# bassamlab/SigmaRL

Measured on AMD Instinct MI355X. Metric: env-steps/sec (agents x envs x steps), CPM scenario, 16 agents (open loop, 32 steps per launch), higher is better.
Workload: dtype f32

## Files before the change

### include/sigmaenv.h

```cpp
#ifndef SIGMAENV_H
#define SIGMAENV_H

#include <stddef.h>
#include <stdint.h>

#ifdef __cplusplus
extern "C" {
#endif

#define SIGMAENV_ABI_VERSION 5

#define SIGMAENV_OK 0
#define SIGMAENV_EINVAL (-22)
#define SIGMAENV_ENOMEM (-12)
#define SIGMAENV_EHIP (-5)
#define SIGMAENV_ENODEV (-19)

#define SIGMAENV_DIST_C2C 0
#define SIGMAENV_DIST_MTV 1

#define SIGMAENV_REW_DISTANCE 1
#define SIGMAENV_REW_TTC 2
#define SIGMAENV_REW_EXACT_SPARSE 4
#define SIGMAENV_REW_HAS_SPARSE 8
// ... 126 lines not shown
                              uint64_t seed, uint64_t counter0, int32_t path_first, int32_t path_count);

int sigmaenv_get(sigmaenv_t* h, sigmaenv_buf_t which, void** dev_ptr, size_t* bytes);

int sigmaenv_set_lanelets(sigmaenv_t* h, int32_t n_lanelets, int32_t max_points, const float* centers, const uint64_t* neighbors);

int sigmaenv_opponent_fill(sigmaenv_t* h, const float* actions);

int sigmaenv_set_slab(sigmaenv_t* h, void* dev_ptr);
int sigmaenv_set_rollout_slab_stride(sigmaenv_t* h, int64_t stride_floats);

int sigmaenv_set_rollout_obs_record(sigmaenv_t* h, float* base, int64_t stride_floats);

int sigmaenv_sync(sigmaenv_t* h);

int sigmaenv_step_time_ms(sigmaenv_t* h, double* avg_ms, int32_t* n_launches);
#define SIGMAENV_KERNEL_STEP 0
#define SIGMAENV_KERNEL_CBF_QP 1
#define SIGMAENV_KERNEL_CBF_MARGIN 2
#define SIGMAENV_KERNEL_MLP32 3
#define SIGMAENV_KERNEL_ACTOR_BF16 4
#define SIGMAENV_KERNEL_COUNT 5
int sigmaenv_kernel_time_ms(sigmaenv_t* h, int32_t kernel_id, double* avg_ms, int32_t* n_launches);

typedef struct sigmaenv_launch_shape {
  int32_t wave_G, wave_wpb, wave_grid, wave_spec, wave_lds_bytes;
  int32_t kern_fastdiv, kern_par, kern_sn, kern_sg, kern_var, kern_mtvs;
  int32_t map_fast_div, pruned_scan;
  int32_t G, block, grid, reset_block, smem_bytes;
  int32_t reserved[2];
} sigmaenv_launch_shape_t;
int sigmaenv_launch_shape(const sigmaenv_t* h, sigmaenv_launch_shape_t* out);

int sigmaenv_trig_selftest(sigmaenv_t* h, int32_t kind, int32_t n, const float* in, float* out);

typedef struct sigmaenv_actor sigmaenv_actor_t;

int sigmaenv_actor_create(int32_t obs_dim, const float* w1, const float* b1, const float* w2, const float* b2, const float* w3, const float* b3,
                          const float* w4, const float* b4, const float* low, const float* high, sigmaenv_actor_t** out);
void sigmaenv_actor_destroy(sigmaenv_actor_t* a);

int sigmaenv_actor_forward(sigmaenv_t* h, sigmaenv_actor_t* a, const float* obs, float* actions, float* log_prob, float* loc_scale, uint64_t seed,
                           uint64_t counter, int32_t deterministic);

typedef struct sigmaenv_mlp32 sigmaenv_mlp32_t;
#define SIGMAENV_MLP32_EXACT 0
#define SIGMAENV_MLP32_SPLIT 1
int sigmaenv_mlp32_set_mode(sigmaenv_mlp32_t* m, int32_t mode);
int sigmaenv_mlp32_get_mode(const sigmaenv_mlp32_t* m);
int sigmaenv_mlp32_create(int32_t n_layers, const int32_t* dims, const float* const* weights, const float* const* biases, sigmaenv_mlp32_t** out);
void sigmaenv_mlp32_destroy(sigmaenv_mlp32_t* m);
int sigmaenv_mlp32_forward(sigmaenv_t* h, sigmaenv_mlp32_t* m, const float* in, int32_t rows, float* out);
int sigmaenv_actor_forward_f32(sigmaenv_t* h, sigmaenv_mlp32_t* m, const float* obs, float* scratch, const float* low, const float* high, float* actions,
                               float* log_prob, float* loc_scale, uint64_t seed, uint64_t counter, int32_t deterministic);

int sigmaenv_mlp32_forward_rows(sigmaenv_t* h, sigmaenv_mlp32_t* m, const float* in, int32_t rows_per_block, int64_t row_stride, int32_t n_blocks, int64_t block_stride,
                                float* out);

int sigmaenv_mlp32_load_device(sigmaenv_t* h, sigmaenv_mlp32_t* m, const float* const* weights_dev, const float* const* biases_dev);
int sigmaenv_actor_load_device(sigmaenv_t* h, sigmaenv_actor_t* a, const float* const* weights_dev, const float* const* biases_dev);

int sigmaenv_mlp32_forward_save(sigmaenv_t* h, sigmaenv_mlp32_t* m, const float* in, int32_t rows_per_block, int64_t row_stride, int32_t n_blocks, int64_t block_stride,
                                float* out, float* acts);
int sigmaenv_mlp32_backward_workspace(const sigmaenv_mlp32_t* m, int64_t rows, uint64_t* n_floats);
int sigmaenv_mlp32_backward(sigmaenv_t* h, sigmaenv_mlp32_t* m, const float* in, int32_t rows_per_block, int64_t row_stride, int32_t n_blocks, int64_t block_stride,
                            const float* acts, const float* dout, float* workspace, float* const* grad_w, float* const* grad_b);
// ... 285 lines not shown
```

### sigmarl_amd/capi.py

```python
from __future__ import annotations

import ctypes as C
import math
import os

ABI_VERSION = 5
DIST_C2C, DIST_MTV = 0, 1
REW_DISTANCE, REW_TTC, REW_EXACT_SPARSE, REW_HAS_SPARSE, REW_CBF, REW_CBF_QP = 1, 2, 4, 8, 16, 32
CBF_MAX_CIRCLES = 4
N_SHORT_TERM = 3
MAX_SHORT_TERM = 8
MAX_NEARING = 4
N_REWARD_INFO = 12

(BUF_STATE, BUF_PREV_POS, BUF_VERTICES, BUF_PATH, BUF_SHORT_TERM, BUF_DIST_REF, BUF_DIST_LEFT, BUF_DIST_RIGHT,
 BUF_DIST_BOUND, BUF_CLOSEST, BUF_DIST_AGENTS, BUF_COL_AGENTS, BUF_COL_FLAGS, BUF_REWARD, BUF_REWARD_INFO, BUF_OBS,
 BUF_NEARING, BUF_DONE, BUF_TIMER, BUF_ACTION, BUF_CBF_NOMINAL) = range(21)

REWARD_INFO_FIELDS = (
    "rew_progress", "rew_reach_goal", "rew_speed", "rew_centerline", "rew_near_other_agents", "rew_near_left_lane",
    "rew_near_right_lane", "rew_collide_other_agents", "rew_collide_lane", "rew_energy_acceleration",
    "rew_energy_steering", "rew_total",
)

# ... 236 lines not shown

_SIGS = {
    "obs_dim": (C.c_int, [C.c_int32]),
    "obs_dim_ex": (C.c_int, [C.c_int32, C.c_int32]),
    "obs_dim_full": (C.c_int, [C.c_int32, C.c_int32, C.c_int32]),
    "n_short_term": (C.c_int, []),
    "create": (C.c_int, [C.POINTER(Config), C.POINTER(Map), C.c_int, C.c_void_p, C.POINTER(C.c_void_p)]),
    "destroy": (None, [C.c_void_p]),
    "last_error": (C.c_char_p, [C.c_void_p]),
    "reset": (C.c_int, [C.c_void_p, C.c_int32, C.c_void_p, C.c_void_p, C.c_void_p, C.c_void_p, C.c_int32]),
    "step": (C.c_int, [C.c_void_p, C.c_void_p]),
    "observe": (C.c_int, [C.c_void_p]),
    "auto_reset": (C.c_int, [C.c_void_p, C.c_uint64, C.c_uint64, C.c_int32, C.c_int32]),
    "get": (C.c_int, [C.c_void_p, C.c_int, C.POINTER(C.c_void_p), C.POINTER(C.c_size_t)]),
    "sync": (C.c_int, [C.c_void_p]),
    "set_lanelets": (C.c_int, [C.c_void_p, C.c_int32, C.c_int32, C.c_void_p, C.c_void_p]),
    "opponent_fill": (C.c_int, [C.c_void_p, C.c_void_p]),
    "set_scenario_lists": (C.c_int, [C.c_void_p, C.c_int32, C.c_void_p, C.c_void_p, C.c_void_p]),
    "cbf_attach": (C.c_int, [C.c_void_p, C.POINTER(CbfConfig), C.c_void_p, C.c_void_p, C.c_int32]),
    "cbf_rewards": (C.c_int, [C.c_void_p, C.c_void_p, C.c_void_p]),
    "cbf_inject_centers": (C.c_int, [C.c_void_p, C.c_void_p]),
    "cbf_qp": (C.c_int, [C.c_void_p, C.c_void_p, C.c_void_p, C.c_void_p, C.c_void_p]),
    "cbf_regroup": (C.c_int, [C.c_void_p]),
    "cbf_get_groups": (C.c_int, [C.c_void_p, C.c_void_p]),
}
_PRODUCT_ONLY = {
    "build_id": (C.c_char_p, []),
    "step_time_ms": (C.c_int, [C.c_void_p, C.POINTER(C.c_double), C.POINTER(C.c_int32)]),
    "kernel_time_ms": (C.c_int, [C.c_void_p, C.c_int32, C.POINTER(C.c_double), C.POINTER(C.c_int32)]),
    "set_slab": (C.c_int, [C.c_void_p, C.c_void_p]),
    "set_rollout_slab_stride": (C.c_int, [C.c_void_p, C.c_int64]),
    "set_rollout_obs_record": (C.c_int, [C.c_void_p, C.c_void_p, C.c_int64]),
    "trig_selftest": (C.c_int, [C.c_void_p, C.c_int32, C.c_int32, C.c_void_p, C.c_void_p]),
    "step_autoreset": (C.c_int, [C.c_void_p, C.c_void_p, C.c_uint64, C.c_uint64, C.c_int32, C.c_int32]),
    "step_autoreset_n": (C.c_int, [C.c_void_p, C.c_void_p, C.c_int32, C.c_int64, C.c_void_p, C.c_int64, C.c_uint64, C.c_uint64, C.c_int32, C.c_int32]),
    "step_autoreset_many": (C.c_int, [C.c_void_p, C.c_int32, C.c_void_p, C.c_void_p, C.c_void_p, C.c_uint64, C.c_int32, C.c_int32]),
    "actor_create": (C.c_int, [C.c_int32] + [C.c_void_p] * 10 + [C.POINTER(C.c_void_p)]),
    "actor_destroy": (None, [C.c_void_p]),
    "actor_forward": (C.c_int, [C.c_void_p, C.c_void_p, C.c_void_p, C.c_void_p, C.c_void_p, C.c_void_p, C.c_uint64, C.c_uint64, C.c_int32]),
    "mlp32_create": (C.c_int, [C.c_int32, C.c_void_p, C.c_void_p, C.c_void_p, C.POINTER(C.c_void_p)]),
    "mlp32_destroy": (None, [C.c_void_p]),
    "mlp32_forward": (C.c_int, [C.c_void_p, C.c_void_p, C.c_void_p, C.c_int32, C.c_void_p]),
    "mlp32_forward_rows": (C.c_int, [C.c_void_p, C.c_void_p, C.c_void_p, C.c_int32, C.c_int64, C.c_int32, C.c_int64, C.c_void_p]),
    "mlp32_set_mode": (C.c_int, [C.c_void_p, C.c_int32]),
    "mlp32_get_mode": (C.c_int, [C.c_void_p]),
    "mlp32_load_device": (C.c_int, [C.c_void_p, C.c_void_p, C.c_void_p, C.c_void_p]),
    "actor_load_device": (C.c_int, [C.c_void_p, C.c_void_p, C.c_void_p, C.c_void_p]),
    "mlp32_forward_save": (C.c_int, [C.c_void_p, C.c_void_p, C.c_void_p, C.c_int32, C.c_int64, C.c_int32, C.c_int64, C.c_void_p, C.c_void_p]),
    "mlp32_backward_workspace": (C.c_int, [C.c_void_p, C.c_int64, C.POINTER(C.c_uint64)]),
    "mlp32_backward": (C.c_int, [C.c_void_p, C.c_void_p, C.c_void_p, C.c_int32, C.c_int64, C.c_int32, C.c_int64, C.c_void_p, C.c_void_p, C.c_void_p, C.c_void_p, C.c_void_p]),
    "mlp32_forward_save_indexed": (C.c_int, [C.c_void_p, C.c_void_p, C.c_void_p, C.c_int32, C.c_int64, C.c_int32, C.c_int64, C.c_void_p, C.c_int32, C.c_void_p, C.c_void_p]),
    "mlp32_backward_indexed": (C.c_int, [C.c_void_p, C.c_void_p, C.c_void_p, C.c_int32, C.c_int64, C.c_int32, C.c_int64, C.c_void_p, C.c_int32, C.c_void_p, C.c_void_p, C.c_void_p,
                                         C.c_void_p, C.c_void_p]),
    "mlp32_forward_rows_pad": (C.c_int, [C.c_void_p, C.c_void_p, C.c_void_p, C.c_int32, C.c_int64, C.c_int32, C.c_int64, C.c_int32, C.c_int32, C.c_void_p]),
    "mlp32_forward_save_indexed_pad": (C.c_int, [C.c_void_p, C.c_void_p, C.c_void_p, C.c_int32, C.c_int64, C.c_int32, C.c_int64, C.c_void_p, C.c_int32, C.c_int32, C.c_int32,
                                                 C.c_void_p, C.c_void_p]),
    "mlp32_backward_indexed_pad": (C.c_int, [C.c_void_p, C.c_void_p, C.c_void_p, C.c_int32, C.c_int64, C.c_int32, C.c_int64, C.c_void_p, C.c_int32, C.c_int32, C.c_int32, C.c_void_p,
                                             C.c_void_p, C.c_void_p, C.c_void_p, C.c_void_p]),
    "ppo_head": (C.c_int, [C.c_void_p, C.POINTER(PpoHeadArgs)]),
    "ppo_head_1d": (C.c_int, [C.c_void_p, C.POINTER(PpoHead1dArgs)]),
    "optim_workspace": (C.c_int, [C.c_void_p, C.POINTER(OptimArgs), C.POINTER(C.c_uint64)]),
    "optim_step": (C.c_int, [C.c_void_p, C.POINTER(OptimArgs)]),
    "mlp32_resolve_mode": (C.c_int, [C.c_void_p, C.c_void_p]),
    "prb_create": (C.c_int, [C.c_void_p, C.c_int64, C.c_double, C.c_double, C.c_double, C.POINTER(C.c_void_p)]),
    "prb_destroy": (None, [C.c_void_p]),
    "prb_extend": (C.c_int, [C.c_void_p, C.c_void_p, C.c_void_p, C.c_int64]),
# ... 119 lines not shown
```

### sigmarl_amd/csrc/sigmaenv.hip

```cpp
#include <hip/hip_runtime.h>

#include <algorithm>
#include <atomic>
#include <cmath>
#include <cstdio>
#include <cstdlib>
#include <cstring>
#include <string>
#include <type_traits>
#include <vector>

#include "sigmaenv_device.h"

using namespace sigmadev;

#ifdef SIGMAENV_PROFILE
#define PROF_TS2(g, tid, k) do { if ((g).dbg_ts2 && (tid) == 0) (g).dbg_ts2[(size_t)blockIdx.x * 16 + (k)] = __builtin_readcyclecounter(); } while (0)
#else
#define PROF_TS2(g, tid, k) do { } while (0)
#endif

#include "../../include/sigmaenv_ref_weights.h"
static_assert(NS >= 1 && NS <= SIGMAENV_MAX_SHORT_TERM, "SIGMAENV_N_SHORT_TERM out of range");
__device__ __constant__ uint32_t W_REF_BITS[NS] = SIGMAENV_W_REF_BITS;
// ... 237 lines not shown
#pragma unroll
    for (int i = 0; i < 4; ++i) e[i] = make_edge(ev[2 * i], ev[2 * i + 1], ev[2 * i + 2], ev[2 * i + 3]);
  }
  r.hit = false;
  boundary_scan<COLLIDE>(lb, nl, lane, cgx, cgy, qv, e, r.dl, r.cp_l, r.hit);
  boundary_scan<COLLIDE>(rb, nr, lane, cgx, cgy, qv, e, r.dr, r.cp_r, r.hit);
  float wh = (float)((double)c.width / 2.0);
  r.dl[0] = r.dl[0] - wh;
  r.dr[0] = r.dr[0] - wh;
}

__device__ __forceinline__ float query_radius(const float* qv, float cgx, float cgy) {
  float R = 0.0f;
#pragma unroll
  for (int q = 0; q < 4; ++q) {
    float ax = qv[2 * q] - cgx, ay = qv[2 * q + 1] - cgy;
    R = fmaxf(R, sqrtf(ax * ax + ay * ay));
  }
  return R * 1.000001f + 1e-6f;
}

__device__ __forceinline__ int nth_set_bit64(unsigned long long m, int c) {
  for (int t = 0; t < c; ++t) m &= (m - 1ull);
  return m ? (__ffsll((long long)m) - 1) : -1;
}
__device__ __forceinline__ bool box_within(const float4 b, float px, float py, float T2) {
  float dx = fmaxf(fmaxf(b.x - px, px - b.z), 0.0f);
  float dy = fmaxf(fmaxf(b.y - py, py - b.w), 0.0f);
  return !((dx * dx + dy * dy) > T2);
}
struct MaskTask {
  int sl, pl, path, k, npt, nch;
  float ax, ay, bx, by;
  unsigned long long nm_tight, nm_near, nm_far;
  int lvl;
  int own;
  const float4* box;
  float px, py, T2;
  unsigned long long rest;
  bool fast;
};
__device__ __forceinline__ void mask_stage1(const DevMap& m, MaskTask& mt, int task, int path, int cp) {
  mt.sl = task / 3; mt.pl = task - mt.sl * 3; mt.path = path;
  const int pl = mt.pl;
  const float* poly = m.center + (size_t)pl * m.poly_stride + (size_t)path * m.P * 2;
  mt.box = m.chunk_box + ((size_t)path * 3 + pl) * m.nch;
  const ulonglong4* neigh = m.chunk_neigh + ((size_t)path * 3 + pl) * m.nch;
  int k = cp - 1;
  k = k < 0 ? 0 : (k > m.P - 2 ? m.P - 2 : k);
  mt.k = k;
  mt.npt = m.n_center[pl * m.n_paths + path];
  const Seg4 sg = load_segment(reinterpret_cast<const float2*>(poly), k);
  mt.ax = sg.ax; mt.ay = sg.ay; mt.bx = sg.bx; mt.by = sg.by;
  const ulonglong4 nm = neigh[k / SIGMAENV_CHUNK];
  mt.nm_tight = nm.x; mt.nm_near = nm.y; mt.nm_far = nm.z;
  mt.own = k / SIGMAENV_CHUNK;
}
template <bool COLLIDE>
__device__ __forceinline__ void mask_stage2(const DevMap& m, const Smem& s, MaskTask& mt, bool stale_first, int N) {
  const int sl = mt.sl, pl = mt.pl, npt = mt.npt;
  if (mt.k > npt - 2) {
    const float* poly = m.center + (size_t)pl * m.poly_stride + (size_t)mt.path * m.P * 2;
    const int k = npt - 2 < 0 ? 0 : npt - 2;
    const Seg4 sg = load_segment(reinterpret_cast<const float2*>(poly), k);
    mt.ax = sg.ax; mt.ay = sg.ay; mt.bx = sg.bx; mt.by = sg.by;
    const ulonglong4 nm = (m.chunk_neigh + ((size_t)mt.path * 3 + pl) * m.nch)[k / SIGMAENV_CHUNK];
    mt.nm_tight = nm.x; mt.nm_near = nm.y; mt.nm_far = nm.z;
    mt.own = k / SIGMAENV_CHUNK;
  }
  const float px = s.st[sl * 8], py = s.st[sl * 8 + 1];
  mt.px = px; mt.py = py;
  const float MARGIN = 1e-4f;
  const float glx = mt.bx - mt.ax, gly = mt.by - mt.ay;
  const float rl2 = __builtin_amdgcn_rcpf(glx * glx + gly * gly);
  float dg;
  {
    const float vx = px - mt.ax, vy = py - mt.ay;
    const float tq = clampf((vx * glx + vy * gly) * rl2, 0.0f, 1.0f);
    const float ex = (mt.ax + glx * tq) - px, ey = (mt.ay + gly * tq) - py;
    dg = __builtin_amdgcn_sqrtf(fmaf(ey, ey, ex * ex)) * 1.000001f + 1e-6f;
  }
  float T = dg;
  if (pl != 0) {
    const bool stale = stale_first && (sl % N == 0);
    const float* qv = stale ? (s.vold + sl * 10) : (s.vnew + sl * 10);
    float w = 0.0f;
#pragma unroll
    for (int j = 0; j < 4; ++j) {
      const float qx = qv[2 * j], qy = qv[2 * j + 1];
      const float vx = qx - mt.ax, vy = qy - mt.ay;
      const float tq = clampf((vx * glx + vy * gly) * rl2, 0.0f, 1.0f);
      const float ex = (mt.ax + glx * tq) - qx, ey = (mt.ay + gly * tq) - qy;
      const float rx = qx - px, ry = qy - py;
      w = fmaxf(w, __builtin_amdgcn_sqrtf(fmaf(ey, ey, ex * ex)) + __builtin_amdgcn_sqrtf(fmaf(ry, ry, rx * rx)));
    }
    T = fmaxf(fmaxf(T, w * 1.000001f + 1e-6f), COLLIDE ? m.rect_radius : 0.0f);
  }
  T += MARGIN;
  mt.T2 = T * T;
  mt.nch = (npt - 1 + SIGMAENV_CHUNK - 1) / SIGMAENV_CHUNK;
  mt.fast = T + dg <= m.neigh_radius_far;
  mt.lvl = mt.fast ? ((T + dg <= m.neigh_radius_tight) ? 0 : ((T + dg <= m.neigh_radius) ? 1 : 2)) : 3;
  mt.rest = mt.fast ? (mt.lvl == 0 ? mt.nm_tight : (mt.lvl == 1 ? mt.nm_near : mt.nm_far)) : 0ull;
}
__device__ __forceinline__ void mask_stage3(const DevMap& m, const Smem& s, MaskTask& mt, int task) {
  const float px = mt.px, py = mt.py, T2 = mt.T2;
  const int nch = mt.nch;
  unsigned long long mk = 0ull;
  unsigned long long rest = mt.rest;
  if (mt.fast && mt.own < nch) { mk |= 1ull << mt.own; rest &= ~(1ull << mt.own); }
  while (rest) {
    int idx[8];
#pragma unroll
    for (int q = 0; q < 8; ++q) { idx[q] = rest ? (__ffsll((long long)rest) - 1) : -1; rest &= rest - 1ull; }
    float4 b[8];
#pragma unroll
    for (int q = 0; q < 8; ++q) b[q] = mt.box[idx[q] < 0 ? 0 : idx[q]];
#pragma unroll
    for (int q = 0; q < 8; ++q) {
      if (idx[q] >= 0 && idx[q] < nch && box_within(b[q], px, py, T2)) mk |= 1ull << idx[q];
    }
  }
  if (!mt.fast) {
    const float4* gbox = m.group_box + ((size_t)mt.path * 3 + mt.pl) * 8;
    unsigned gm = 0u;
#pragma unroll
    for (int gidx = 0; gidx < 8; ++gidx) {
      if (gidx * 8 < nch && box_within(gbox[gidx], px, py, T2)) gm |= 1u << gidx;
    }
    while (gm) {
      const int gidx = __ffs((int)gm) - 1;
      gm &= gm - 1u;
#pragma unroll
      for (int q = 0; q < 8; ++q) {
        const int cidx = gidx * 8 + q;
        if (cidx < nch && box_within(mt.box[cidx], px, py, T2)) mk |= 1ull << cidx;
      }
    }
  }
  s.npts[task] = mt.npt;
  s.cmask[task] = mk;
  uint8_t* cl = s.cand + task * CAND_LIST;
  for (int j = 0; mk && j < CAND_LIST; ++j) {
    cl[j] = (uint8_t)(__ffsll((long long)mk) - 1);
    mk &= mk - 1ull;
  }
}
template <bool COLLIDE>
__device__ inline void scan_mask_task(const DevMap& m, const Smem& s, int task, bool stale_first, int N) {
  MaskTask mt;
  mask_stage1(m, mt, task, s.path[task / 3], s.cp[task]);
  mask_stage2<COLLIDE>(m, s, mt, stale_first, N);
  mask_stage3(m, s, mt, task);
}

// ... 1293 lines not shown
  while (G > 1 && (B + G - 1) / G < 4 * n_cu) G >>= 1;
  return G;
}

#ifdef SIGMAENV_POISON
__global__ void sigma_poison_probe_kernel(unsigned* out) {
  extern __shared__ char probe_smem[];
  if (threadIdx.x == 0) { probe_smem[0] = 1; out[0] = sigma_lds_alloc_units() + (probe_smem[0] ? 0u : 1u); }
}
static int poison_probe(hipStream_t stream) {
  static bool done = false;
  if (done) return SIGMAENV_OK;
  unsigned* d = nullptr;
  unsigned units[2] = {0u, 0u};
  if (hipMalloc((void**)&d, 8) != hipSuccess) return SIGMAENV_ENOMEM;
  hipLaunchKernelGGL(sigma_poison_probe_kernel, dim3(1), dim3(64), 32768, stream, d);
  hipLaunchKernelGGL(sigma_poison_probe_kernel, dim3(1), dim3(64), 16384, stream, d + 1);
  if (hipMemcpyAsync(units, d, 8, hipMemcpyDeviceToHost, stream) != hipSuccess || hipStreamSynchronize(stream) != hipSuccess) { (void)hipFree(d); return SIGMAENV_EHIP; }
  (void)hipFree(d);
  unsigned granule = 0u;
  for (unsigned g : {64u, 128u, 256u, 512u})
    if (units[0] * g >= 32768u && units[0] * g < 32768u + 2048u && units[1] * g >= 16384u && units[1] * g < 16384u + 2048u) granule = g;
  if (granule == 0u) {
    fprintf(stderr, "sigmaenv (poison build): unexpected LDS_ALLOC.LDS_SIZE readings %u / %u for 32768 / 16384 bytes\n", units[0], units[1]);
    return SIGMAENV_EHIP;
  }
  if (hipMemcpyToSymbol(HIP_SYMBOL(sigmadev::sigma_lds_granule), &granule, sizeof(unsigned)) != hipSuccess) return SIGMAENV_EHIP;
  fprintf(stderr, "sigmaenv (poison build): LDS and scratch buffers are poisoned (LDS_SIZE unit = %u bytes)\n", granule);
  done = true;
  return SIGMAENV_OK;
}
#endif

extern "C" int sigmaenv_create(const sigmaenv_config_t* cfg, const sigmaenv_map_t* map, int device_id, void* hip_stream, sigmaenv_t** out) {
  if (!cfg || !map || !out) return SIGMAENV_EINVAL;
  *out = nullptr;
  if (cfg->abi_version != SIGMAENV_ABI_VERSION) return SIGMAENV_EINVAL;
  for (int k = 0; k < 3; ++k) if (cfg->reserved[k] != 0) return SIGMAENV_EINVAL;
  if (cfg->n_points_short_term != 0 && cfg->n_points_short_term != NS) {
    fprintf(stderr, "sigmaenv_create: n_points_short_term = %d, but this library is built for %d (make -C sigmarl_amd/csrc NS=%d)\n", cfg->n_points_short_term, NS, cfg->n_points_short_term);
    return SIGMAENV_EINVAL;
  }
  if (cfg->env_index_base < 0 || !(cfg->obs_noise_level >= 0.0f)) return SIGMAENV_EINVAL;
  if (cfg->n_envs < 1 || cfg->n_agents < 1 || cfg->n_agents > SIGMAENV_MAX_AGENTS) return SIGMAENV_EINVAL;
  if (cfg->n_nearing < 0 || cfg->n_nearing > SIGMAENV_MAX_NEARING || cfg->n_nearing > cfg->n_agents - 1) return SIGMAENV_EINVAL;
  if (cfg->distance_type != SIGMAENV_DIST_C2C && cfg->distance_type != SIGMAENV_DIST_MTV) return SIGMAENV_EINVAL;
  if (map->n_paths < 1 || map->stride_points < 2) return SIGMAENV_EINVAL;
  int n_dev = 0;
  if (hipGetDeviceCount(&n_dev) != hipSuccess || n_dev < 1 || device_id < 0 || device_id >= n_dev) return SIGMAENV_ENODEV;
  if (hipSetDevice(device_id) != hipSuccess) return SIGMAENV_ENODEV;
#ifdef SIGMAENV_POISON
  { const int rcp = poison_probe(reinterpret_cast<hipStream_t>(hip_stream)); if (rcp != SIGMAENV_OK) return rcp; }
#endif
  sigmaenv* h = new sigmaenv();
  h->cfg = *cfg;
  h->device = device_id;
  h->stream = reinterpret_cast<hipStream_t>(hip_stream);
  const int B = h->B = cfg->n_envs, N = h->N = cfg->n_agents, K = h->K = cfg->n_nearing;
  h->D = sigmaenv_obs_dim_full(N, K, cfg->obs_flags);
  if (h->D < 0) { delete h; return SIGMAENV_EINVAL; }
  h->DL = h->D;
  if (cfg->obs_flags != 0) {
    const ObsLayout L(cfg->obs_flags, N, K);
    if (L.D != h->D) { delete h; return SIGMAENV_EINVAL; }
    h->DL = L.DL;
  }
// ... 39 lines not shown
#define ALLOC(ptr, bytes)                                         \
  if ((rc = dev_alloc(h, (void**)&(ptr), (bytes))) != SIGMAENV_OK) { \
    std::string e = h->err;                                       \
    sigmaenv_destroy(h);                                          \
    fprintf(stderr, "sigmaenv_create: %s\n", e.c_str());        \
    return rc;                                                    \
  }
  float *d_c, *d_l, *d_r, *d_y;
  int32_t *d_nc, *d_nl, *d_nr;
  uint8_t* d_loop;
  ALLOC(d_c, hc.size() * 4 * 3); d_l = d_c + hc.size(); d_r = d_l + hc.size();
  ALLOC(d_y, (size_t)np * S * 4);
  ALLOC(d_nc, (size_t)np * 4 * 3); d_nl = d_nc + np; d_nr = d_nl + np;
  ALLOC(d_loop, (size_t)np);
#define H2D(dst, src, bytes)                                                                     \
  if (hipMemcpyAsync((dst), (src), (bytes), hipMemcpyHostToDevice, h->stream) != hipSuccess) {   \
    sigmaenv_destroy(h);                                                                         \
    return SIGMAENV_EHIP;                                                                        \
  }
  H2D(d_c, hc.data(), hc.size() * 4); H2D(d_l, hl.data(), hl.size() * 4); H2D(d_r, hr.data(), hr.size() * 4);
  H2D(d_y, map->yaw, (size_t)np * S * 4);
  H2D(d_nc, map->n_center, (size_t)np * 4); H2D(d_nl, map->n_left, (size_t)np * 4); H2D(d_nr, map->n_right, (size_t)np * 4);
  H2D(d_loop, map->is_loop, (size_t)np);
  int nch = (P - 1 + SIGMAENV_CHUNK - 1) / SIGMAENV_CHUNK;
  int real_nch = 0;
  for (int p = 0; p < np; ++p) {
    const int longest = std::max(map->n_center[p], std::max(map->n_left[p], map->n_right[p]));
    real_nch = std::max(real_nch, (longest - 1 + SIGMAENV_CHUNK - 1) / SIGMAENV_CHUNK);
  }
  bool prune = real_nch <= 64;
  if (const char* e = getenv("SIGMAENV_PRUNE")) prune = prune && atoi(e) != 0;
  float4 *d_box = nullptr, *d_gbox = nullptr;
  std::vector<float4> hb, hg;
  std::vector<ulonglong4> hn;
  ulonglong4* d_neigh = nullptr;
  const float neigh_radius_far = 9.0f * (sqrtf((float)((double)cfg->length / 2.0) * (float)((double)cfg->length / 2.0) +
                                               (float)((double)cfg->width / 2.0) * (float)((double)cfg->width / 2.0)) * 1.00001f + 1e-5f);
  const float neigh_radius_tight = 3.6f * (sqrtf((float)((double)cfg->length / 2.0) * (float)((double)cfg->length / 2.0) +
                                                 (float)((double)cfg->width / 2.0) * (float)((double)cfg->width / 2.0)) * 1.00001f + 1e-5f);
  const float neigh_radius = 6.0f * (sqrtf((float)((double)cfg->length / 2.0) * (float)((double)cfg->length / 2.0) +
                                           (float)((double)cfg->width / 2.0) * (float)((double)cfg->width / 2.0)) * 1.00001f + 1e-5f);
  if (prune) {
    hb.assign((size_t)np * 3 * nch, make_float4(1e30f, 1e30f, -1e30f, -1e30f));
    for (int p = 0; p < np; ++p) {
      const float* polys[3] = {hc.data() + (size_t)p * P * 2, hl.data() + (size_t)p * P * 2, hr.data() + (size_t)p * P * 2};
      const int cnt[3] = {map->n_center[p], map->n_left[p], map->n_right[p]};
      for (int q = 0; q < 3; ++q) {
        for (int k = 0; k + 1 < cnt[q]; ++k) {
          float4& bx = hb[((size_t)p * 3 + q) * nch + k / SIGMAENV_CHUNK];
          for (int e2 = 0; e2 < 2; ++e2) {
            float x = polys[q][2 * (k + e2)], y = polys[q][2 * (k + e2) + 1];
            bx.x = x < bx.x ? x : bx.x; bx.y = y < bx.y ? y : bx.y; bx.z = x > bx.z ? x : bx.z; bx.w = y > bx.w ? y : bx.w;
          }
        }
      }
    }
    ALLOC(d_box, hb.size() * sizeof(float4));
    H2D(d_box, hb.data(), hb.size() * sizeof(float4));
    hg.assign((size_t)np * 3 * 8, make_float4(1e30f, 1e30f, -1e30f, -1e30f));
    for (size_t pq = 0; pq < (size_t)np * 3; ++pq) {
      for (int cidx = 0; cidx < nch; ++cidx) {
        const float4& bx = hb[pq * nch + cidx];
        if (bx.x > bx.z) continue;
        float4& gx = hg[pq * 8 + cidx / 8];
        gx.x = bx.x < gx.x ? bx.x : gx.x; gx.y = bx.y < gx.y ? bx.y : gx.y; gx.z = bx.z > gx.z ? bx.z : gx.z; gx.w = bx.w > gx.w ? bx.w : gx.w;
      }
    }
    ALLOC(d_gbox, hg.size() * sizeof(float4));
    H2D(d_gbox, hg.data(), hg.size() * sizeof(float4));
    hn.assign((size_t)np * 3 * nch, make_ulonglong4(0ull, 0ull, 0ull, 0ull));
    for (size_t pq = 0; pq < (size_t)np * 3; ++pq) {
      for (int a = 0; a < nch; ++a) {
        const float4& A = hb[pq * nch + a];
        if (A.x > A.z) continue;
        unsigned long long bits = 0ull, bits_far = 0ull, bits_tight = 0ull;
        for (int b2 = 0; b2 < nch; ++b2) {
          const float4& Bx = hb[pq * nch + b2];
          if (Bx.x > Bx.z) continue;
          double dx = std::max(std::max((double)A.x - Bx.z, (double)Bx.x - A.z), 0.0);
          double dy = std::max(std::max((double)A.y - Bx.w, (double)Bx.y - A.w), 0.0);
          const double dd = std::sqrt(dx * dx + dy * dy);
          if (dd <= (double)neigh_radius_tight + 1e-5) bits_tight |= 1ull << b2;
          if (dd <= (double)neigh_radius + 1e-5) bits |= 1ull << b2;
          if (dd <= (double)neigh_radius_far + 1e-5) bits_far |= 1ull << b2;
        }
        hn[pq * nch + a] = make_ulonglong4(bits_tight, bits, bits_far, 0ull);
      }
    }
    ALLOC(d_neigh, hn.size() * sizeof(ulonglong4));
    H2D(d_neigh, hn.data(), hn.size() * sizeof(ulonglong4));
  }
  const float lh = (float)((double)cfg->length / 2.0), wh = (float)((double)cfg->width / 2.0);
  const float rect_radius = sqrtf(lh * lh + wh * wh) * 1.00001f + 1e-5f;
  int fast_div = 1;
  for (int p = 0; p < np && fast_div; ++p) {
    const float* polys[3] = {hc.data() + (size_t)p * P * 2, hl.data() + (size_t)p * P * 2, hr.data() + (size_t)p * P * 2};
    const int cnt[3] = {map->n_center[p], map->n_left[p], map->n_right[p]};
    for (int q = 0; q < 3 && fast_div; ++q) {
      for (int k = 0; k + 1 < cnt[q]; ++k) {
        const float lx = polys[q][2 * (k + 1)] - polys[q][2 * k], ly = polys[q][2 * (k + 1) + 1] - polys[q][2 * k + 1];
        const float len2 = lx * lx + ly * ly;
        if (!(len2 >= 0x1p-60f && len2 <= 0x1p60f)) { fast_div = 0; break; }
      }
    }
  }
  if (const char* e = getenv("SIGMAENV_FASTDIV")) fast_div = fast_div && atoi(e) != 0;
  h->map = DevMap{d_c, d_l, d_r, d_y, d_nc, d_nl, d_nr, d_loop, P, np, S, d_box, d_gbox, d_neigh, neigh_radius, neigh_radius_far, prune ? nch : 0, nullptr, fast_div, rect_radius, (int32_t)hc.size()};
  h->map.neigh_radius_tight = neigh_radius_tight;
  {
    float* d_tab = nullptr;
    ALLOC(d_tab, (size_t)np * P * START_ROW * sizeof(float));
    const size_t tab_smem = Smem::bytes(64, 1, 0, 1) + 16;
    if (tab_smem > 64 * 1024)
      (void)hipFuncSetAttribute(reinterpret_cast<const void*>(sigmaenv_start_table_kernel), hipFuncAttributeMaxDynamicSharedMemorySize, (int)tab_smem);
    hipLaunchKernelGGL(sigmaenv_start_table_kernel, dim3((np * P + 63) / 64), dim3(256), tab_smem, h->stream, h->cfg, h->map, d_tab);
    if (hipGetLastError() != hipSuccess) { sigmaenv_destroy(h); return SIGMAENV_EHIP; }
    h->map.start_table = d_tab;
  }
  const size_t BN = (size_t)B * N;
  DevBufs& g = h->buf;
  struct Spec { int id; void** p; size_t bytes; };
  Spec specs[] = {
      {SIGMAENV_BUF_STATE, (void**)&g.state, BN * 32}, {SIGMAENV_BUF_PREV_POS, (void**)&g.prev_pos, BN * 8},
// ... 529 lines not shown
```

### sigmarl_amd/csrc/sigmaenv_device.h

```cpp
#pragma once

#include <hip/hip_runtime.h>
#include <stdint.h>

#include "../../include/sigmaenv.h"
#include "../../include/sigma_trig_f32.h"
#include "sigmaenv_dist.h"

#define NS SIGMAENV_N_SHORT_TERM
#define PI32 3.14159274101257324f
#define TWO_PI32 (2.0f * PI32)

namespace sigmadev {

#ifdef SIGMAENV_POISON
__device__ unsigned sigma_lds_granule = 0u;
__device__ __forceinline__ unsigned sigma_lds_alloc_units() { return (unsigned)__builtin_amdgcn_s_getreg(6 | (12 << 6) | ((9 - 1) << 11)); }
__device__ __forceinline__ void sigma_poison_lds() {
  const unsigned words = sigma_lds_alloc_units() * sigma_lds_granule / 4u;
  auto* lds = (__attribute__((address_space(3))) unsigned*)0;
  const unsigned tid = threadIdx.x + blockDim.x * (threadIdx.y + blockDim.y * threadIdx.z), nt = blockDim.x * blockDim.y * blockDim.z;
  for (unsigned k = tid; k < words; k += nt) lds[k] = 0xFFFFFFFFu;
  __syncthreads();
}
#else
__device__ __forceinline__ void sigma_poison_lds() {}
#endif

struct DevMap {
  const float* center;
  const float* left;
  const float* right;
  const float* yaw;
  const int32_t* n_center;
  const int32_t* n_left;
  const int32_t* n_right;
  const uint8_t* is_loop;
  int32_t P, n_paths, yaw_stride;
  const float4* chunk_box;
  const float4* group_box;
  const ulonglong4* chunk_neigh;
  float neigh_radius, neigh_radius_far;
  int32_t nch;
  const float* start_table;
  int32_t fast_div;
  float rect_radius;
  int32_t poly_stride;
  int32_t n_lists;
  float cdf0, cdf1, cdf2;
  float neigh_radius_tight;
  unsigned long long list_first16, list_count16;
};
#define SIGMAENV_CHUNK 4
struct CfgDerived {
  float l_wb;
  float k_beta;
  float lh, wh;
  float diag;
  float rew_denom;
  float r_pos, r_v, r_dl;
  float r_wx, r_wy;
  float min_d_sq;
};
struct DevConfig {
  sigmaenv_config_t c;
  CfgDerived d;
};
inline CfgDerived derive_config(const sigmaenv_config_t& c) {
  CfgDerived d;
  d.l_wb = (float)((double)c.l_f + (double)c.l_r);
  d.k_beta = (float)((double)c.l_r / ((double)c.l_f + (double)c.l_r));
  d.lh = (float)((double)c.length / 2.0);
  d.wh = (float)((double)c.width / 2.0);
  const float xx = c.world_x_dim * c.world_x_dim, yy = c.world_y_dim * c.world_y_dim;
// ... 418 lines not shown
```

### sigmarl_amd/csrc/sigmaenv_step_wave.inc

```

__device__ __forceinline__ float dpp_swap1(float v) {
  return __int_as_float(__builtin_amdgcn_update_dpp(0, __float_as_int(v), 0xB1, 0xF, 0xF, true));
}

__device__ __forceinline__ void bicycle_step_pair(const sigmaenv_config_t& c, const CfgDerived& dv, float s[8], float u0, float u1, float uc[2], float cs_yaw[2], bool par, int h, float cr[3]) {
  const float a0 = clampf(u0, -c.max_speed, c.max_speed);
  const float a1 = clampf(u1, -c.max_steering, c.max_steering);
  uc[0] = a0;
  uc[1] = a1;
  float x = s[0], y = s[1], psi = s[2], v = s[3], delta = s[4];
  float u_acc = (a0 - v) / c.dt;
  float u_sr = (a1 - delta) / c.dt;
  u_acc = clampf(u_acc, c.min_acc, c.max_acc);
  u_sr = clampf(u_sr, c.min_steering_rate, c.max_steering_rate);
  const float l_wb = dv.l_wb, k_beta = dv.k_beta;
  const float dt = c.dt;
  float delta_new = delta + dt * u_sr;
  delta_new = remainder_pos(delta_new + PI32, TWO_PI32) - PI32;
  float tan_d, beta, beta1, tan_new;
  {
    const float x1 = (par && h) ? delta_new : delta;
    const float t1 = cr_tan(x1);
    const float b1 = cr_atan(k_beta * t1);
    if (par) {
// ... 209 lines not shown
    const int incl = wave_inclusive_sum(cnt, lane);
    int slot = near_total + incl - cnt;
    near_total += __builtin_amdgcn_readlane(incl, 63);
#pragma unroll
    for (int u = 0; u < SIGMAENV_CHUNK; ++u) {
      if ((nb >> u) & 1u) {
        if (slot < near_cap) s.nearl[slot] = (uint16_t)(code0 + u);
        if (slot < xy_cap) s.nearxy[slot] = make_float4(sg[u].ax, sg[u].ay, sg[u].bx, sg[u].by);
        ++slot;
      }
    }
  };
  for (int base = 0; base < n_tasks; base += 64) {
    const int tl = base + lane;
    const int grp_raw = fdiv(tl, g.mSG), sl_raw = tl - grp_raw * SG;
    const int pl_raw = grp_raw >= 2 ? 0 : grp_raw + 1;
    const int tpm = pl_raw * SG + sl_raw;
    const bool act = tl < n_tasks && sl_raw < slots;
    const int pl = act ? pl_raw : 0, sl = act ? sl_raw : 0;
    const int task = sl * 3 + pl;
    unsigned long long mk = 0ull;
#ifdef SIGMAENV_PROFILE
    int lvl_prof = 0;
#endif
    if (act) {
      MaskTask mt;
      mask_stage1(m, mt, task, s.path[sl], s.cp[task]);
      mask_stage2<true>(m, s, mt, true, N);
#ifdef SIGMAENV_PROFILE
      lvl_prof = mt.lvl;
#endif
      const float px = mt.px, py = mt.py, T2 = mt.T2;
      const int nch = mt.nch;
      unsigned long long rest = mt.rest;
      if (mt.fast && mt.own < nch) { mk |= 1ull << mt.own; rest &= ~(1ull << mt.own); }
      while (rest) {
        int idx[8];
#pragma unroll
        for (int q = 0; q < 8; ++q) { idx[q] = rest ? (__ffsll((long long)rest) - 1) : -1; rest &= rest - 1ull; }
        float4 b[8];
#pragma unroll
        for (int q = 0; q < 8; ++q) b[q] = mt.box[idx[q] < 0 ? 0 : idx[q]];
#pragma unroll
        for (int q = 0; q < 8; ++q) {
          if (idx[q] >= 0 && idx[q] < nch && box_within(b[q], px, py, T2)) mk |= 1ull << idx[q];
        }
      }
      if (!mt.fast) {
        const float4* gbox = m.group_box + ((size_t)mt.path * 3 + pl) * 8;
        unsigned gm = 0u;
#pragma unroll 1
        for (int gidx = 0; gidx < 8; ++gidx) {
          if (gidx * 8 < nch && box_within(gbox[gidx], px, py, T2)) gm |= 1u << gidx;
        }
        while (gm) {
          const int gidx = __ffs((int)gm) - 1;
          gm &= gm - 1u;
#pragma unroll 1
          for (int q = 0; q < 8; ++q) {
            const int cidx = gidx * 8 + q;
            if (cidx < nch && box_within(mt.box[cidx], px, py, T2)) mk |= 1ull << cidx;
          }
        }
      }
      s.npts[task] = mt.npt;
      s.acc64[task] = ~0ull;
      if (pl != 0) {
        const int bt = sl * 2 + (pl - 1);
        uint32_t* a = s.acc32 + bt * 4;
        a[0] = 0x7F800000u; a[1] = 0x7F800000u; a[2] = 0x7F800000u; a[3] = 0x7F800000u;
        s.nearn[bt] = 0;
      }
    }
#ifdef SIGMAENV_PROFILE
    if (g.dbg_ts && lane == 0 && base == 0) g.dbg_ts[(size_t)t.env0 / (size_t)G * 16 + 10] = __builtin_readcyclecounter();
    {
      const unsigned long long bfar = __ballot(act && lvl_prof >= 2), btight = __ballot(act && lvl_prof == 0);
#ifndef SIGMAENV_PROFILE_RT
      if (g.dbg_ts && lane == 0) {
        unsigned long long* row = g.dbg_ts + (size_t)t.env0 / (size_t)G * 16;
// ... 771 lines not shown
```

Baseline: 3.249 billion.

## Replace neighbour chunk bitmasks with precomputed ring-ordered index lists

```diff
diff --git a/include/sigmaenv.h b/include/sigmaenv.h
--- a/include/sigmaenv.h
+++ b/include/sigmaenv.h
@@ -182,6 +182,8 @@
 } sigmaenv_launch_shape_t;
 int sigmaenv_launch_shape(const sigmaenv_t* h, sigmaenv_launch_shape_t* out);
 
+int sigmaenv_neigh_rows(const float* boxes, int32_t nch, float length, float width, uint8_t* rows, uint64_t* masks);
+
 int sigmaenv_trig_selftest(sigmaenv_t* h, int32_t kind, int32_t n, const float* in, float* out);
 
 typedef struct sigmaenv_actor sigmaenv_actor_t;
diff --git a/sigmarl_amd/capi.py b/sigmarl_amd/capi.py
--- a/sigmarl_amd/capi.py
+++ b/sigmarl_amd/capi.py
@@ -292,6 +292,7 @@
     "set_rollout_slab_stride": (C.c_int, [C.c_void_p, C.c_int64]),
     "set_rollout_obs_record": (C.c_int, [C.c_void_p, C.c_void_p, C.c_int64]),
     "trig_selftest": (C.c_int, [C.c_void_p, C.c_int32, C.c_int32, C.c_void_p, C.c_void_p]),
+    "neigh_rows": (C.c_int, [C.c_void_p, C.c_int32, C.c_float, C.c_float, C.c_void_p, C.c_void_p]),
     "step_autoreset": (C.c_int, [C.c_void_p, C.c_void_p, C.c_uint64, C.c_uint64, C.c_int32, C.c_int32]),
     "step_autoreset_n": (C.c_int, [C.c_void_p, C.c_void_p, C.c_int32, C.c_int64, C.c_void_p, C.c_int64, C.c_uint64, C.c_uint64, C.c_int32, C.c_int32]),
     "step_autoreset_many": (C.c_int, [C.c_void_p, C.c_int32, C.c_void_p, C.c_void_p, C.c_void_p, C.c_uint64, C.c_int32, C.c_int32]),
diff --git a/sigmarl_amd/csrc/sigmaenv.hip b/sigmarl_amd/csrc/sigmaenv.hip
--- a/sigmarl_amd/csrc/sigmaenv.hip
+++ b/sigmarl_amd/csrc/sigmaenv.hip
@@ -293,28 +293,66 @@
 struct MaskTask {
   int sl, pl, path, k, npt, nch;
   float ax, ay, bx, by;
-  unsigned long long nm_tight, nm_near, nm_far;
+  uint4 row_lo, row_hi;
   int lvl;
   int own;
   const float4* box;
   float px, py, T2;
-  unsigned long long rest;
+  int cnt;
+  bool own_within;
   bool fast;
 };
+__device__ __forceinline__ void neigh_row_load(const DevMap& m, MaskTask& mt, int chunk) {
+  const uint4* r = reinterpret_cast<const uint4*>(m.chunk_neigh + (((size_t)mt.path * 3 + mt.pl) * m.nch + chunk));
+  mt.row_lo = r[0]; mt.row_hi = r[1];
+}
+__device__ __forceinline__ void neigh_list_select(MaskTask& mt, int lvl) {
+  const uint32_t cw = mt.row_hi.w;
+  const uint32_t cnt = (cw >> (8 * (lvl & 3))) & 0xFFu;
+  const bool marked = cnt == NEIGH_OVERFLOW;
+  mt.lvl = marked ? 3 : lvl;
+  mt.fast = lvl < 3 && !marked;
+  mt.cnt = marked ? 0 : (int)cnt;
+}
+template <int POS0, int WIDTH>
+__device__ __forceinline__ void neigh_round(const DevMap& m, const MaskTask& mt, unsigned row0, unsigned long long& mk) {
+  const uint32_t word[8] = {mt.row_lo.x, mt.row_lo.y, mt.row_lo.z, mt.row_lo.w, mt.row_hi.x, mt.row_hi.y, mt.row_hi.z, mt.row_hi.w};
+  const char* const base = reinterpret_cast<const char*>(m.chunk_box);
+  unsigned idx[WIDTH];
+  float4 b[WIDTH];
+#pragma unroll
+  for (int q = 0; q < WIDTH; ++q) {
+    idx[q] = (word[(POS0 + q) / 4] >> (8 * ((POS0 + q) % 4))) & 0xFFu;
+    b[q] = *reinterpret_cast<const float4*>(base + (size_t)(row0 + idx[q] * (unsigned)sizeof(float4)));
+  }
+#pragma unroll
+  for (int q = 0; q < WIDTH; ++q) mk |= (unsigned long long)box_within(b[q], mt.px, mt.py, mt.T2) << idx[q];
+}
+__device__ __forceinline__ unsigned long long neigh_candidates(const DevMap& m, const MaskTask& mt) {
+  unsigned long long mk = 0ull;
+  const unsigned row0 = (unsigned)((mt.path * 3 + mt.pl) * m.nch) * (unsigned)sizeof(float4);
+  if (0 < mt.cnt) neigh_round<0, 8>(m, mt, row0, mk);
+  if (8 < mt.cnt) neigh_round<8, 4>(m, mt, row0, mk);
+  if (12 < mt.cnt) neigh_round<12, 4>(m, mt, row0, mk);
+  if (16 < mt.cnt) {
+    neigh_round<16, 4>(m, mt, row0, mk);
+    if (20 < mt.cnt) neigh_round<20, 4>(m, mt, row0, mk);
+    if (24 < mt.cnt) neigh_round<24, 4>(m, mt, row0, mk);
+  }
+  return mk;
+}
 __device__ __forceinline__ void mask_stage1(const DevMap& m, MaskTask& mt, int task, int path, int cp) {
   mt.sl = task / 3; mt.pl = task - mt.sl * 3; mt.path = path;
   const int pl = mt.pl;
   const float* poly = m.center + (size_t)pl * m.poly_stride + (size_t)path * m.P * 2;
   mt.box = m.chunk_box + ((size_t)path * 3 + pl) * m.nch;
-  const ulonglong4* neigh = m.chunk_neigh + ((size_t)path * 3 + pl) * m.nch;
   int k = cp - 1;
   k = k < 0 ? 0 : (k > m.P - 2 ? m.P - 2 : k);
   mt.k = k;
   mt.npt = m.n_center[pl * m.n_paths + path];
   const Seg4 sg = load_segment(reinterpret_cast<const float2*>(poly), k);
   mt.ax = sg.ax; mt.ay = sg.ay; mt.bx = sg.bx; mt.by = sg.by;
-  const ulonglong4 nm = neigh[k / SIGMAENV_CHUNK];
-  mt.nm_tight = nm.x; mt.nm_near = nm.y; mt.nm_far = nm.z;
+  neigh_row_load(m, mt, k / SIGMAENV_CHUNK);
   mt.own = k / SIGMAENV_CHUNK;
 }
 template <bool COLLIDE>
@@ -325,8 +363,7 @@
     const int k = npt - 2 < 0 ? 0 : npt - 2;
     const Seg4 sg = load_segment(reinterpret_cast<const float2*>(poly), k);
     mt.ax = sg.ax; mt.ay = sg.ay; mt.bx = sg.bx; mt.by = sg.by;
-    const ulonglong4 nm = (m.chunk_neigh + ((size_t)mt.path * 3 + pl) * m.nch)[k / SIGMAENV_CHUNK];
-    mt.nm_tight = nm.x; mt.nm_near = nm.y; mt.nm_far = nm.z;
+    neigh_row_load(m, mt, k / SIGMAENV_CHUNK);
     mt.own = k / SIGMAENV_CHUNK;
   }
   const float px = s.st[sl * 8], py = s.st[sl * 8 + 1];
@@ -360,28 +397,14 @@
   T += MARGIN;
   mt.T2 = T * T;
   mt.nch = (npt - 1 + SIGMAENV_CHUNK - 1) / SIGMAENV_CHUNK;
-  mt.fast = T + dg <= m.neigh_radius_far;
-  mt.lvl = mt.fast ? ((T + dg <= m.neigh_radius_tight) ? 0 : ((T + dg <= m.neigh_radius) ? 1 : 2)) : 3;
-  mt.rest = mt.fast ? (mt.lvl == 0 ? mt.nm_tight : (mt.lvl == 1 ? mt.nm_near : mt.nm_far)) : 0ull;
+  mt.own_within = T + dg <= m.neigh_radius_far;
+  neigh_list_select(mt, mt.own_within ? ((T + dg <= m.neigh_radius_tight) ? 0 : ((T + dg <= m.neigh_radius) ? 1 : 2)) : 3);
 }
 __device__ __forceinline__ void mask_stage3(const DevMap& m, const Smem& s, MaskTask& mt, int task) {
   const float px = mt.px, py = mt.py, T2 = mt.T2;
   const int nch = mt.nch;
-  unsigned long long mk = 0ull;
-  unsigned long long rest = mt.rest;
-  if (mt.fast && mt.own < nch) { mk |= 1ull << mt.own; rest &= ~(1ull << mt.own); }
-  while (rest) {
-    int idx[8];
-#pragma unroll
-    for (int q = 0; q < 8; ++q) { idx[q] = rest ? (__ffsll((long long)rest) - 1) : -1; rest &= rest - 1ull; }
-    float4 b[8];
-#pragma unroll
-    for (int q = 0; q < 8; ++q) b[q] = mt.box[idx[q] < 0 ? 0 : idx[q]];
-#pragma unroll
-    for (int q = 0; q < 8; ++q) {
-      if (idx[q] >= 0 && idx[q] < nch && box_within(b[q], px, py, T2)) mk |= 1ull << idx[q];
-    }
-  }
+  unsigned long long mk = neigh_candidates(m, mt);
+  if (mt.own_within && mt.own < nch) mk |= 1ull << mt.own;
   if (!mt.fast) {
     const float4* gbox = m.group_box + ((size_t)mt.path * 3 + mt.pl) * 8;
     unsigned gm = 0u;
@@ -1741,6 +1764,22 @@
 }
 #endif
 
+extern "C" int sigmaenv_neigh_rows(const float* boxes, int32_t nch, float length, float width, uint8_t* rows, uint64_t* masks) {
+  if (!boxes || !rows || nch < 1 || nch > 64) return SIGMAENV_EINVAL;
+  float radius[3];
+  neigh_radii(length, width, radius);
+  std::vector<NeighRow> r((size_t)nch);
+  std::vector<unsigned long long> mk((size_t)nch * 3);
+  std::vector<float4> bx((size_t)nch);
+  for (int c = 0; c < nch; ++c) bx[c] = make_float4(boxes[4 * c], boxes[4 * c + 1], boxes[4 * c + 2], boxes[4 * c + 3]);
+  neigh_rows_build(bx.data(), nch, radius, r.data(), mk.data());
+  memcpy(rows, r.data(), r.size() * sizeof(NeighRow));
+  if (masks) {
+    for (size_t i = 0; i < mk.size(); ++i) masks[i] = (uint64_t)mk[i];
+  }
+  return SIGMAENV_OK;
+}
+
 extern "C" int sigmaenv_create(const sigmaenv_config_t* cfg, const sigmaenv_map_t* map, int device_id, void* hip_stream, sigmaenv_t** out) {
   if (!cfg || !map || !out) return SIGMAENV_EINVAL;
   *out = nullptr;
@@ -1846,14 +1885,11 @@
   if (const char* e = getenv("SIGMAENV_PRUNE")) prune = prune && atoi(e) != 0;
   float4 *d_box = nullptr, *d_gbox = nullptr;
   std::vector<float4> hb, hg;
-  std::vector<ulonglong4> hn;
-  ulonglong4* d_neigh = nullptr;
-  const float neigh_radius_far = 9.0f * (sqrtf((float)((double)cfg->length / 2.0) * (float)((double)cfg->length / 2.0) +
-                                               (float)((double)cfg->width / 2.0) * (float)((double)cfg->width / 2.0)) * 1.00001f + 1e-5f);
-  const float neigh_radius_tight = 3.6f * (sqrtf((float)((double)cfg->length / 2.0) * (float)((double)cfg->length / 2.0) +
-                                                 (float)((double)cfg->width / 2.0) * (float)((double)cfg->width / 2.0)) * 1.00001f + 1e-5f);
-  const float neigh_radius = 6.0f * (sqrtf((float)((double)cfg->length / 2.0) * (float)((double)cfg->length / 2.0) +
-                                           (float)((double)cfg->width / 2.0) * (float)((double)cfg->width / 2.0)) * 1.00001f + 1e-5f);
+  std::vector<NeighRow> hn;
+  NeighRow* d_neigh = nullptr;
+  float radius[3];
+  neigh_radii(cfg->length, cfg->width, radius);
+  const float neigh_radius_tight = radius[0], neigh_radius = radius[1], neigh_radius_far = radius[2];
   if (prune) {
     hb.assign((size_t)np * 3 * nch, make_float4(1e30f, 1e30f, -1e30f, -1e30f));
     for (int p = 0; p < np; ++p) {
@@ -1882,27 +1918,10 @@
     }
     ALLOC(d_gbox, hg.size() * sizeof(float4));
     H2D(d_gbox, hg.data(), hg.size() * sizeof(float4));
-    hn.assign((size_t)np * 3 * nch, make_ulonglong4(0ull, 0ull, 0ull, 0ull));
-    for (size_t pq = 0; pq < (size_t)np * 3; ++pq) {
-      for (int a = 0; a < nch; ++a) {
-        const float4& A = hb[pq * nch + a];
-        if (A.x > A.z) continue;
-        unsigned long long bits = 0ull, bits_far = 0ull, bits_tight = 0ull;
-        for (int b2 = 0; b2 < nch; ++b2) {
-          const float4& Bx = hb[pq * nch + b2];
-          if (Bx.x > Bx.z) continue;
-          double dx = std::max(std::max((double)A.x - Bx.z, (double)Bx.x - A.z), 0.0);
-          double dy = std::max(std::max((double)A.y - Bx.w, (double)Bx.y - A.w), 0.0);
-          const double dd = std::sqrt(dx * dx + dy * dy);
-          if (dd <= (double)neigh_radius_tight + 1e-5) bits_tight |= 1ull << b2;
-          if (dd <= (double)neigh_radius + 1e-5) bits |= 1ull << b2;
-          if (dd <= (double)neigh_radius_far + 1e-5) bits_far |= 1ull << b2;
-        }
-        hn[pq * nch + a] = make_ulonglong4(bits_tight, bits, bits_far, 0ull);
-      }
-    }
-    ALLOC(d_neigh, hn.size() * sizeof(ulonglong4));
-    H2D(d_neigh, hn.data(), hn.size() * sizeof(ulonglong4));
+    hn.resize((size_t)np * 3 * nch);
+    for (size_t pq = 0; pq < (size_t)np * 3; ++pq) neigh_rows_build(hb.data() + pq * nch, nch, radius, hn.data() + pq * nch, nullptr);
+    ALLOC(d_neigh, hn.size() * sizeof(NeighRow));
+    H2D(d_neigh, hn.data(), hn.size() * sizeof(NeighRow));
   }
   const float lh = (float)((double)cfg->length / 2.0), wh = (float)((double)cfg->width / 2.0);
   const float rect_radius = sqrtf(lh * lh + wh * wh) * 1.00001f + 1e-5f;
diff --git a/sigmarl_amd/csrc/sigmaenv_device.h b/sigmarl_amd/csrc/sigmaenv_device.h
--- a/sigmarl_amd/csrc/sigmaenv_device.h
+++ b/sigmarl_amd/csrc/sigmaenv_device.h
@@ -2,6 +2,9 @@
 
 #include <hip/hip_runtime.h>
 #include <stdint.h>
+
+#include <algorithm>
+#include <cmath>
 
 #include "../../include/sigmaenv.h"
 #include "../../include/sigma_trig_f32.h"
@@ -26,6 +29,59 @@
 #else
 __device__ __forceinline__ void sigma_poison_lds() {}
 #endif
+
+#define NEIGH_CAP 28
+#define NEIGH_OVERFLOW 0xFFu
+struct alignas(16) NeighRow {
+  uint8_t list[NEIGH_CAP];
+  uint8_t cnt[3];
+  uint8_t pad;
+};
+static_assert(sizeof(NeighRow) == 32, "NeighRow is two 16-byte loads");
+inline void neigh_radii(float length, float width, float radius[3]) {
+  const float lh = (float)((double)length / 2.0), wh = (float)((double)width / 2.0);
+  const float r = sqrtf(lh * lh + wh * wh) * 1.00001f + 1e-5f;
+  radius[0] = 3.6f * r; radius[1] = 6.0f * r; radius[2] = 9.0f * r;
+}
+inline void neigh_rows_build(const float4* box, int nch, const float radius[3], NeighRow* rows, unsigned long long* masks) {
+  for (int a = 0; a < nch; ++a) {
+    NeighRow r{};
+    unsigned long long bits[3] = {0ull, 0ull, 0ull};
+    const float4& A = box[a];
+    if (!(A.x > A.z)) {
+      for (int b = 0; b < nch; ++b) {
+        const float4& B = box[b];
+        if (B.x > B.z) continue;
+        const double dx = std::max(std::max((double)A.x - B.z, (double)B.x - A.z), 0.0);
+        const double dy = std::max(std::max((double)A.y - B.w, (double)B.y - A.w), 0.0);
+        const double dd = std::sqrt(dx * dx + dy * dy);
+        for (int l = 0; l < 3; ++l) {
+          if (dd <= (double)radius[l] + 1e-5) bits[l] |= 1ull << b;
+        }
+      }
+    }
+    int n = 0;
+    for (int l = 0; l < 3; ++l) {
+      const unsigned long long ring = bits[l] & ~(l ? bits[l - 1] : 0ull) & ~(1ull << (a & 63));
+      const int len = n + __builtin_popcountll(ring);
+      if (n == (int)NEIGH_OVERFLOW || len > NEIGH_CAP) {
+        n = NEIGH_OVERFLOW;
+      } else {
+        for (int b = 0; b < nch && b < 64; ++b) {
+          if ((ring >> b) & 1ull) r.list[n++] = (uint8_t)b;
+        }
+      }
+      r.cnt[l] = (uint8_t)n;
+      if (masks) masks[a * 3 + l] = bits[l];
+    }
+    int stored = 0;
+    for (int l = 0; l < 3; ++l) {
+      if (r.cnt[l] != NEIGH_OVERFLOW) stored = r.cnt[l];
+    }
+    for (int j2 = stored; j2 < NEIGH_CAP && stored > 0; ++j2) r.list[j2] = r.list[stored - 1];
+    rows[a] = r;
+  }
+}
 
 struct DevMap {
   const float* center;
@@ -39,7 +95,7 @@
   int32_t P, n_paths, yaw_stride;
   const float4* chunk_box;
   const float4* group_box;
-  const ulonglong4* chunk_neigh;
+  const NeighRow* chunk_neigh;
   float neigh_radius, neigh_radius_far;
   int32_t nch;
   const float* start_table;
diff --git a/sigmarl_amd/csrc/sigmaenv_step_wave.inc b/sigmarl_amd/csrc/sigmaenv_step_wave.inc
--- a/sigmarl_amd/csrc/sigmaenv_step_wave.inc
+++ b/sigmarl_amd/csrc/sigmaenv_step_wave.inc
@@ -265,20 +265,8 @@
 #endif
       const float px = mt.px, py = mt.py, T2 = mt.T2;
       const int nch = mt.nch;
-      unsigned long long rest = mt.rest;
-      if (mt.fast && mt.own < nch) { mk |= 1ull << mt.own; rest &= ~(1ull << mt.own); }
-      while (rest) {
-        int idx[8];
-#pragma unroll
-        for (int q = 0; q < 8; ++q) { idx[q] = rest ? (__ffsll((long long)rest) - 1) : -1; rest &= rest - 1ull; }
-        float4 b[8];
-#pragma unroll
-        for (int q = 0; q < 8; ++q) b[q] = mt.box[idx[q] < 0 ? 0 : idx[q]];
-#pragma unroll
-        for (int q = 0; q < 8; ++q) {
-          if (idx[q] >= 0 && idx[q] < nch && box_within(b[q], px, py, T2)) mk |= 1ull << idx[q];
-        }
-      }
+      mk = neigh_candidates(m, mt);
+      if (mt.own_within && mt.own < nch) mk |= 1ull << mt.own;
       if (!mt.fast) {
         const float4* gbox = m.group_box + ((size_t)mt.path * 3 + pl) * 8;
         unsigned gm = 0u;
```

Result: faster. 3.396 billion (median of 6 runs) (+4.5%).
